# gmarcais/Jellyfish

Measured on AMD Instinct MI355X. Metric: k-mers/sec at k=21 canonical, 150 bp synthetic reads, bit-exact counts, higher is better.
Workload: dtype u64

## Files before the change

### jellyfish_amd/csrc/kernels.hip.hpp

```cpp
#pragma once
#include <hip/hip_runtime.h>
#include <stdint.h>
#include "kmer_core.hpp"

namespace jfgpu {

constexpr int kBlock = 256;
constexpr int kPerThread = kPerLane;
constexpr int kTilePos = kBlock * kPerThread;

enum Counter : int { CTR_FULL = 0, CTR_MERS = 1, CTR_OVF_FULL = 2, CTR_OVF_USED = 3, CTR_MISROUTED = 4, CTR_DIRECT = 5,
                     CTR_T_ITEMS = 6, CTR_T_QUEUED = 7 ,
                     CTR_PROF0 = 8 , CTR_COUNT = 12 };

#ifdef JFGPU_PHASE_PROF
__device__ unsigned long long g_phase_prof[24];
struct PhaseClk {
  long long acc[8] = {0, 0, 0, 0, 0, 0, 0, 0}; long long t;
  __device__ PhaseClk() { t = clock64(); }
  __device__ void mark(int i) { const long long n = clock64(); acc[i] += n - t; t = n; }
  __device__ void flush(int base) { if(threadIdx.x == 0) for(int i = 0; i < 8; ++i) if(acc[i]) atomicAdd(&g_phase_prof[base + i], (unsigned long long)acc[i]); }
};
#define JF_PHASE(pc, i) (pc).mark(i)
#define JF_PHASE_FLUSH(pc, base) (pc).flush(base)
// ... 4 lines not shown
#endif

struct DevBloom {
  uint32_t* data;
  uint64_t m;
  uint64_t recip;
  uint32_t nh;
  uint32_t nbytes;
  uint32_t kind;
  uint32_t pad_;
  const uint64_t* tbl1;
  const uint64_t* tbl2;
  uint64_t* cache;
  uint64_t cache_mask;
};

struct DevTable {
  TableGeom g;
  uint64_t* slots;
  const uint64_t* fwd_tbl;
  const uint64_t* inv_tbl;
  uint64_t* ovf_key;
  uint64_t* ovf_cnt;
  uint64_t ovf_mask;
  uint64_t* counters;
  uint32_t max_probe;
  DevBloom bloom;
  uint8_t* dirty;
};

#if defined(JFGPU_EMU)
__device__ __forceinline__ void lds_barrier() { __syncthreads(); }
#define JF_DYN_LDS(name) unsigned char* name = ::hip_emu::dyn_lds()
#else
__device__ __forceinline__ void lds_barrier() { asm volatile("s_waitcnt lgkmcnt(0)\n\ts_barrier" ::: "memory"); }
#define JF_DYN_LDS(name) extern __shared__ __align__(16) unsigned char name[]
#endif

__device__ inline bool bloom_admits(const DevBloom& B, uint64_t key);
__device__ inline uint32_t bloom_admit_mask(const DevBloom& B, const TableGeom& g, const LaneWords& L);

__device__ inline void ovf_add(const DevTable& T, uint64_t slot, uint64_t units) {
  const uint64_t want = slot + 1;
  uint64_t h = (slot * 0x9E3779B97F4A7C15ull) >> 20;
  for(uint64_t p = 0; p <= T.ovf_mask; ++p) {
    const uint64_t s = (h + p) & T.ovf_mask;
    unsigned long long old = atomicCAS((unsigned long long*)&T.ovf_key[s], 0ull, (unsigned long long)want);
    if(old == 0ull) atomicAdd((unsigned long long*)&T.counters[CTR_OVF_USED], 1ull);
    if(old == 0ull || old == want) {
      atomicAdd((unsigned long long*)&T.ovf_cnt[s], (unsigned long long)units);
      return;
    }
  }
  atomicAdd((unsigned long long*)&T.counters[CTR_OVF_FULL], 1ull);
}

__device__ inline uint64_t ovf_get(const DevTable& T, uint64_t slot) {
  const uint64_t want = slot + 1;
  uint64_t h = (slot * 0x9E3779B97F4A7C15ull) >> 20;
  for(uint64_t p = 0; p <= T.ovf_mask; ++p) {
    const uint64_t s = (h + p) & T.ovf_mask;
    const uint64_t k = T.ovf_key[s];
    if(k == 0) return 0;
    if(k == want) return T.ovf_cnt[s];
  }
  return 0;
}

__device__ inline uint64_t full_count(const DevTable& T, uint64_t word, uint64_t slot, bool have_ovf) {
// ... 892 lines not shown
```

### jellyfish_amd/csrc/kernels_bloom_part.hip.hpp

```cpp
#pragma once
#include "kernels_part.hip.hpp"
#include "kernels_p1ring.hip.hpp"
#include "kernels_bloom.hip.hpp"

namespace jfgpu {

constexpr uint32_t kBloomSegBits = 16;
constexpr uint32_t kBloomItemLow = kBloomSegBits + 3;
constexpr int kBloomPer = 10;
constexpr int kBloomChunk = kPBlock * kBloomPer;

struct BloomPart {
  uint32_t b1, b2;
  uint32_t n_seg;
  uint32_t pad_;
};

__device__ inline void bloom_item_direct(const DevBloom& B, const BloomPart& BP, uint32_t bucket, uint32_t item) {
  const uint64_t seg = ((uint64_t)bucket << BP.b2) | (item >> kBloomItemLow);
  const uint64_t byte = (seg << kBloomSegBits) | ((item >> 3) & 0xFFFFu);
  bloom_bump(B.data, byte, item & 7u);
}

struct BloomDirect {
// ... 132 lines not shown
                                                                   unsigned int* __restrict__ gcur, unsigned long long* __restrict__ tot,
                                                                   uint32_t* __restrict__ out, unsigned long long* __restrict__ mers) {
  p1_bloom_granule_body<NB, kBloomPer, false>(B, BP, g, base, lo, hi, cap, gcur, tot, out, mers);
}
template <int NB>
__global__ __launch_bounds__(kPBlock) __attribute__((amdgpu_waves_per_eu(8, 8)))
void p1_bloom_granule2_kernel(DevBloom B, BloomPart BP, TableGeom g, const uint8_t* __restrict__ base,
                              int64_t lo, int64_t hi, uint32_t cap,
                              unsigned int* __restrict__ gcur, unsigned long long* __restrict__ tot,
                              uint32_t* __restrict__ out, unsigned long long* __restrict__ mers) {
  p1_bloom_granule_body<NB, 5, true>(B, BP, g, base, lo, hi, cap, gcur, tot, out, mers);
}


constexpr uint32_t kBloomRingBytes = 256;
__device__ __attribute__((noinline)) void bloom_p1_item_direct_call(uint32_t* data, uint32_t b2, uint32_t bucket, uint32_t item) {
  const uint64_t seg = ((uint64_t)bucket << b2) | (item >> kBloomItemLow);
  const uint64_t byte = (seg << kBloomSegBits) | ((item >> 3) & 0xFFFFu);
  bloom_bump(data, byte, item & 7u);
}
struct BloomP1RingDirect {
  static constexpr bool kCountsDirect = false;
  uint32_t* data; uint32_t b2;
  __device__ void operator()(uint32_t bucket, uint64_t item, uint32_t cnt) const { for(uint32_t i = 0; i < cnt; ++i) bloom_p1_item_direct_call(data, b2, bucket, (uint32_t)item); }
};

template <int NB, int PER>
__global__ __launch_bounds__(kPBlock) void p1_bloom_ring_kernel(DevBloom B, BloomPart BP, TableGeom g, BloomP1RingDirect D, const uint8_t* __restrict__ base,
                                                                int64_t lo, int64_t hi, uint32_t cap,
                                                                unsigned int* __restrict__ gcur, unsigned long long* __restrict__ tot,
                                                                uint32_t* __restrict__ out, unsigned long long* __restrict__ mers,
                                                                uint64_t* __restrict__ strag, uint32_t* __restrict__ strag_n) {
  using R = Ring<uint32_t, kBloomRingBytes>;
  JF_DYN_LDS(s_dyn);
  const uint32_t nb = 1u << BP.b1;
  uint32_t* s_ring = reinterpret_cast<uint32_t*>(s_dyn);
  uint4* s_tn = reinterpret_cast<uint4*>(s_dyn + (size_t)nb * kBloomRingBytes + kBloomRingBytes);
  __shared__ uint32_t s_fill[kGranMaxB + 32];
  __shared__ uint32_t s_nstrag;
  __shared__ uint32_t s_codes[kPBlock + 2];
  __shared__ uint32_t s_inv[kPBlock + 2];
  const uint32_t t = threadIdx.x, lane = t & 63;
  const bool owner = t < nb;
  for(uint32_t i = t; i < B.nbytes * 32; i += blockDim.x) {
    const uint32_t j = i >> 4, v = i & 15u;
    const uint32_t at = (j >> 1) * 256 + ((j & 1) ? (v << 4) : v);
    const uint64_t a = B.tbl1[at], c = B.tbl2[at];
    s_tn[i] = make_uint4((uint32_t)a, (uint32_t)(a >> 32), (uint32_t)c, (uint32_t)(c >> 32));
  }
  ring_init<uint32_t, kBloomRingBytes>(s_ring, s_fill, nb, &s_nstrag);
  const uint32_t dump = nb * R::kSlots + (lane & (R::kSlots - 1));
  unsigned int* const gshort = gcur + nb;
  uint64_t* const my_strag = strag + (size_t)blockIdx.x * kStragPerBlock;
  const uint32_t k = g.k, rc_shift = 2 * (k - 1);
  const uint32_t sub_mask = (1u << BP.b2) - 1u;
  RingBooks Bk;
  if(owner) { Bk.nxt = atomicAdd(&gcur[t], kGran); Bk.nxt_asked = true; }
  uint32_t* const my_region = out + (uint64_t)t * cap;
  uint32_t my_mers = 0;
  auto straggler = [&](uint32_t b, uint32_t item, uint32_t cnt) {
    const uint32_t at = atomicAdd(&s_nstrag, 1u);
    if(at < kStragPerBlock) strag_store<uint32_t>(my_strag + at, b, item, cnt);
    else D(b, (uint64_t)item, cnt);
  };
  const int64_t n_tiles = (hi + kPTilePos - 1) / kPTilePos;
  TileRaw Rw = tile_fetch(base, (int64_t)blockIdx.x * kPTilePos, lo, hi);
  lds_barrier();
  for(int64_t tile = blockIdx.x; tile < n_tiles; tile += gridDim.x) {
    const LaneWords L = tile_stage(Rw, tile * kPTilePos, lo, hi, s_codes, s_inv);
    Rw = tile_fetch(base, (tile + gridDim.x) * kPTilePos, lo, hi);
    uint64_t fw = (((uint64_t)L.p2 << 32) | L.p1) & g.key_mask;
    uint64_t rc = revcomp64(fw, k);
    uint64_t smear = L.inv48;
    for(uint32_t s = 1; s < k; ) { const uint32_t step = s < k - s ? s : k - s; smear |= smear >> step; s += step; }
    const uint32_t vmask = ~(uint32_t)smear & 0xFFFFu;
    my_mers += (uint32_t)__popc(vmask);
#pragma unroll 1
    for(int j = 0; j < kPerLane; ++j) {
      const uint64_t c = (L.cur >> (2 * (15 - j))) & 3u;
      fw = ((fw << 2) | c) & g.key_mask;
      rc = (rc >> 2) | ((3ull - c) << rc_shift);
      const bool valid = (vmask >> (15 - j)) & 1u;
      const uint64_t key = (g.canonical && rc < fw) ? rc : fw;
      uint32_t a0 = 0, a1 = 0, c0 = 0, c1 = 0;
      constexpr int kNibs = NB ? 2 * NB : 16;
#pragma unroll
      for(int q = 0; q < kNibs; ++q)
        if(NB || (uint32_t)q < 2 * B.nbytes) { const uint4 e = s_tn[q * 16 + ((uint32_t)(key >> (4 * q)) & 15u)]; a0 ^= e.x; a1 ^= e.y; c0 ^= e.z; c1 ^= e.w; }
      uint64_t cell = bloom_mod(((uint64_t)a1 << 32) | a0, B.m, B.recip);
      const uint64_t inc = bloom_mod(((uint64_t)c1 << 32) | c0, B.m, B.recip);
      for(uint32_t h0 = 0; h0 < B.nh; h0 += PER) {
        uint32_t ea[PER], eo[PER], ei[PER];
#pragma unroll
        for(int e = 0; e < PER; ++e) {
          const bool on = valid && h0 + e < B.nh;
          uint64_t byte; uint32_t dig;
          divmod5(cell, byte, dig);
          const uint32_t seg = (uint32_t)(byte >> kBloomSegBits);
          const uint32_t b = seg >> BP.b2;
          ei[e] = ((seg & sub_mask) << kBloomItemLow) | ((uint32_t)(byte & 0xFFFFu) << 3) | dig;
          const uint32_t o = atomicAdd(&s_fill[on ? b : nb + (lane & 31u)], 1u);
          ea[e] = on ? b * R::kSlots : dump; eo[e] = on ? o : 0u;
          cell += inc; if(cell >= B.m) cell -= B.m;
        }
        uint32_t ghosts = 0;
#pragma unroll
        for(int e = 0; e < PER; ++e) {
          const uint32_t full = eo[e] & R::kFull;
          ghosts |= full;
          const uint32_t at = ea[e] + ((eo[e] + (eo[e] >> 16)) & (R::kSlots - 1));
          s_ring[full ? dump : at] = ei[e];
        }
        if(ghosts) {
#pragma unroll 1
          for(int e = 0; e < PER; ++e) if(eo[e] & R::kFull) straggler(ea[e] / R::kSlots, ei[e], 1u);
        }
        lds_barrier();
        wave_prio<3>();
        if(owner) ring_flush<uint32_t, false, kBloomRingBytes>(s_ring, s_fill, t, false, Bk, my_region, cap, gcur, gshort, straggler);
        wave_prio<0>();
#ifdef JFGPU_BLOOM_P1_BAR2
        lds_barrier();
#endif
      }
    }
  }
  lds_barrier();
  if(owner) { ring_flush<uint32_t, false, kBloomRingBytes>(s_ring, s_fill, t, true, Bk, my_region, cap, gcur, gshort, straggler); ring_finish<uint32_t>(Bk, t, my_region, cap, gshort, tot); }
  lds_barrier();
  if(t == 0) strag_n[blockIdx.x] = s_nstrag < kStragPerBlock ? s_nstrag : kStragPerBlock;
  uint64_t w = my_mers;
  for(int o = 32; o > 0; o >>= 1) w += __shfl_down(w, o, 64);
  if((threadIdx.x & 63) == 0 && w) atomicAdd(mers, (unsigned long long)w);
}

__device__ inline void bloom_lds_bump(uint32_t* s_seg, uint32_t item) {
  const uint32_t off = (item >> 3) & 0xFFFFu, dig = item & 7u;
  uint32_t* w = s_seg + (off >> 2);
  const uint32_t sh = 8 * (off & 3);
  const uint32_t add = bloom_pow3(dig) << sh;
  uint32_t old = *w;
  while(true) {
    if(bloom_digit((old >> sh) & 0xFFu, dig) >= 2) return;
    const uint32_t seen = atomicCAS(w, old, old + add);
    if(seen == old) return;
    old = seen;
  }
}
// ... 53 lines not shown
```

### jellyfish_amd/csrc/kernels_p1ring.hip.hpp

```cpp
#pragma once
#include <type_traits>
#include "kernels_part.hip.hpp"

namespace jfgpu {

template <int P> __device__ __forceinline__ void wave_prio() {
#if defined(__HIP_DEVICE_COMPILE__)
  __builtin_amdgcn_s_setprio(P);
#endif
}

__device__ __forceinline__ uint32_t adm_to_vmask(uint32_t adm) {
  uint32_t r = 0;
#pragma unroll
  for(int j = 0; j < 16; ++j) r |= ((adm >> j) & 1u) << (15 - j);
  return r;
}


constexpr uint32_t kStragPerBlock = 16384;

template <typename ITEM, uint32_t RB = 128> struct Ring {
  static constexpr uint32_t kSlots = RB / sizeof(ITEM);
  static constexpr uint32_t kUnit = 64 / sizeof(ITEM);
  static constexpr uint32_t kChunk = 16 / sizeof(ITEM);
  static constexpr uint32_t kFull = 0xFFFFu & ~(kSlots - 1);
  static constexpr uint32_t kWords = sizeof(ITEM) <= 4 ? 1 : 1 + sizeof(ITEM) / 8;
  __device__ static uint32_t first_fill(uint32_t b) { return ((kChunk * b) & (kSlots - 1)) << 16; }
};

template <typename ITEM> __device__ __forceinline__ uint32_t chunk_hole_key(const uint4& v) {
  if constexpr(sizeof(ITEM) == 4) { const uint32_t a = v.x > v.y ? v.x : v.y, c = v.z > v.w ? v.z : v.w; return a > c ? a : c; }
  else if constexpr(sizeof(ITEM) == 8) { const uint32_t a = v.x & v.y, c = v.z & v.w; return a > c ? a : c; }
  else return v.x & v.y & v.z & v.w;
}
template <typename ITEM, typename F> __device__ __forceinline__ void chunk_items(const uint4& v, F&& f) {
  if constexpr(sizeof(ITEM) == 4) { f((ITEM)v.x); f((ITEM)v.y); f((ITEM)v.z); f((ITEM)v.w); }
  else if constexpr(sizeof(ITEM) == 8) { f((ITEM)(((uint64_t)v.y << 32) | v.x)); f((ITEM)(((uint64_t)v.w << 32) | v.z)); }
  else f((ITEM)(((unsigned __int128)(((uint64_t)v.w << 32) | v.z) << 64) | (((uint64_t)v.y << 32) | v.x)));
}

template <typename ITEM> __device__ __forceinline__ void strag_store(uint64_t* rec, uint32_t b, ITEM item, uint32_t cnt) {
  const uint64_t meta = ((uint64_t)(cnt < 255u ? cnt : 255u) << 56) | ((uint64_t)(b & 0xFFFFFFu) << 32);
  if constexpr(sizeof(ITEM) == 4) rec[0] = meta | (uint32_t)item;
  else if constexpr(sizeof(ITEM) == 8) { rec[0] = meta; rec[1] = (uint64_t)item; }
  else { rec[0] = meta; rec[1] = (uint64_t)item; rec[2] = (uint64_t)(item >> 64); }
}
template <typename ITEM> __device__ __forceinline__ void strag_load(const uint64_t* rec, uint32_t& b, ITEM& item, uint32_t& cnt) {
  const uint64_t meta = rec[0];
  b = (uint32_t)(meta >> 32) & 0xFFFFFFu; cnt = (uint32_t)(meta >> 56);
  if constexpr(sizeof(ITEM) == 4) item = (ITEM)(uint32_t)meta;
  else if constexpr(sizeof(ITEM) == 8) item = (ITEM)rec[1];
  else item = (ITEM)(((unsigned __int128)rec[2] << 64) | rec[1]);
}

struct RingBooks { uint32_t gpos = 0, room = 0, nxt = 0, stored = 0; bool nxt_asked = false, exhausted = false; };

template <typename ITEM, bool OWNED = false, uint32_t RB = 128, typename STRAG>
__device__ __forceinline__ void ring_flush(ITEM* s_ring, uint32_t* s_fill, uint32_t t, bool all, RingBooks& B, ITEM* my_region, uint32_t cap,
                                           unsigned int* gcur, unsigned int* gshort, STRAG&& straggler) {
  using R = Ring<ITEM, RB>;
  const ITEM hole = (ITEM)~(ITEM)0;
  const uint32_t w = s_fill[t];
  uint32_t cnt = w & 0xFFFFu; if(cnt > R::kSlots) cnt = R::kSlots;
  const uint32_t rb = (w >> 16) & (R::kSlots - 1);
  uint32_t units = cnt / R::kUnit; if(all && (cnt % R::kUnit)) ++units;
  uint32_t nout = 0;
  for(uint32_t s = 0; s < units; ++s) {
    uint4 v[4];
    const uint32_t s0 = (rb + s * R::kUnit) & (R::kSlots - 1);
#pragma unroll
    for(int q = 0; q < 4; ++q) v[q] = *reinterpret_cast<const uint4*>(s_ring + t * R::kSlots + ((s0 + R::kChunk * q) & (R::kSlots - 1)));
    if(!all) {
      uint32_t mx = 0;
#pragma unroll
      for(int q = 0; q < 4; ++q) { const uint32_t a = chunk_hole_key<ITEM>(v[q]); mx = mx > a ? mx : a; }
      if(mx == 0xFFFFFFFFu) break;
    }
    if constexpr(!OWNED) {
    if(B.room == 0 && B.nxt_asked) {
      if((uint64_t)B.nxt + kGran <= cap) { B.gpos = B.nxt; B.room = kGran; }
      else { B.exhausted = true; if(B.nxt < cap) atomicMax(&gshort[t], cap - B.nxt); }
      B.nxt_asked = false;
    }
    if(B.room == 0 && !B.exhausted) {
      const uint32_t r0 = atomicAdd(&gcur[t], kGran);
      if((uint64_t)r0 + kGran <= cap) { B.gpos = r0; B.room = kGran; }
      else { B.exhausted = true; if(r0 < cap) atomicMax(&gshort[t], cap - r0); }
    }
    }
    if(B.room) {
      uint4* dst = reinterpret_cast<uint4*>(my_region + B.gpos);
#pragma unroll
      for(int q = 0; q < 4; ++q) dst[q] = v[q];
      const uint32_t real = cnt - s * R::kUnit < R::kUnit ? cnt - s * R::kUnit : R::kUnit;
      B.gpos += OWNED ? real : R::kUnit; B.room -= R::kUnit; B.stored += real;
    } else {
#pragma unroll
      for(int q = 0; q < 4; ++q) chunk_items<ITEM>(v[q], [&](ITEM x) { if(x != hole) straggler(t, x, 1u); });
    }
#pragma unroll
    for(int q = 0; q < 4; ++q)
      *reinterpret_cast<uint4*>(s_ring + t * R::kSlots + ((s0 + R::kChunk * q) & (R::kSlots - 1))) = make_uint4(0xFFFFFFFFu, 0xFFFFFFFFu, 0xFFFFFFFFu, 0xFFFFFFFFu);
    ++nout;
  }
  if constexpr(!OWNED) { if(!all && !B.nxt_asked && !B.exhausted && B.room < R::kSlots) { B.nxt = atomicAdd(&gcur[t], kGran); B.nxt_asked = true; } }
  uint32_t expect = w;
  while(nout || (expect & 0xFFFFu) > R::kSlots) {
    uint32_t c = expect & 0xFFFFu; if(c > R::kSlots) c = R::kSlots;
    const uint32_t taken = nout * R::kUnit < c ? nout * R::kUnit : c;
    const uint32_t neww = ((((expect >> 16) + nout * R::kUnit) & 0xFFFFu) << 16) | (c - taken);
    const uint32_t old = atomicCAS(&s_fill[t], expect, neww);
    if(old == expect) break;
    expect = old;
  }
}

template <typename ITEM, uint32_t RB = 128>
__device__ __forceinline__ void ring_init(ITEM* s_ring, uint32_t* s_fill, uint32_t nb, uint32_t* s_nstrag) {
  using R = Ring<ITEM, RB>;
  for(uint32_t j = threadIdx.x; j < nb; j += blockDim.x) s_fill[j] = R::first_fill(j);
  uint4* r4 = reinterpret_cast<uint4*>(s_ring);
  for(uint32_t j = threadIdx.x; j < nb * (RB / 16) + RB / 16; j += blockDim.x) r4[j] = make_uint4(0xFFFFFFFFu, 0xFFFFFFFFu, 0xFFFFFFFFu, 0xFFFFFFFFu);
  if(threadIdx.x == 0) *s_nstrag = 0;
}

template <typename ITEM>
__device__ __forceinline__ void ring_finish(const RingBooks& B, uint32_t t, ITEM* my_region, uint32_t cap, unsigned int* gshort, unsigned long long* tot) {
  const ITEM hole = (ITEM)~(ITEM)0;
  for(uint32_t r = 0; r < B.room; ++r) my_region[B.gpos + r] = hole;
  if(B.nxt_asked) {
    if((uint64_t)B.nxt + kGran <= cap) { for(uint32_t r = 0; r < kGran; ++r) my_region[B.nxt + r] = hole; }
    else if(B.nxt < cap) atomicMax(&gshort[t], cap - B.nxt);
  }
  if(tot && B.stored) atomicAdd(&tot[t], (unsigned long long)B.stored);
}

struct OneWordDirect {
  static constexpr bool kCountsDirect = true;
  const DevTable* Tm; uint32_t b2; int returning;
  __device__ void operator()(uint32_t b, uint64_t item, uint32_t cnt) const { item_direct_call(Tm, b2, b, item, cnt, returning); }
};
struct RouteListDirect {
  static constexpr bool kCountsDirect = false;
  StragList SL;
  __device__ void operator()(uint32_t b, uint64_t item, uint32_t cnt) const {
    for(uint32_t i = 0; i < cnt; ++i) { const unsigned long long at = atomicAdd(SL.n, 1ull); if(at < SL.cap) SL.rec[at] = ((uint64_t)b << 32) | (uint32_t)item; }
  }
};

template <typename ITEM, bool BLOOM, int NB, int CANON, typename DIRECT = OneWordDirect>
__global__ __launch_bounds__(kPBlock) void p1_ring_kernel(DevTable T, DIRECT D, PartGeom P, const uint8_t* __restrict__ base,
                                                          int64_t lo, int64_t hi, uint32_t cap,
                                                          unsigned int* __restrict__ gcur,
                                                          unsigned long long* __restrict__ tot,
                                                          ITEM* __restrict__ out,
                                                          uint64_t* __restrict__ strag, uint32_t* __restrict__ strag_n) {
  using R = Ring<ITEM>;
  constexpr int RP = sizeof(ITEM) == 4 ? 8 : 4;
  JF_DYN_LDS(s_dyn);
  ITEM* s_ring = reinterpret_cast<ITEM*>(s_dyn);
  __shared__ uint64_t s_fwd[NB < 0 ? 1 : 8 * 256];
  __shared__ uint32_t s_fill[kGranMaxB + 32];
  __shared__ uint32_t s_nstrag;
  __shared__ uint32_t s_codes[kPBlock + 2];
  __shared__ uint32_t s_inv[kPBlock + 2];
  const TableGeom& g = T.g;
  const uint32_t nb = 1u << P.b1;
  const uint32_t t = threadIdx.x, lane = t & 63;
  const bool owner = t < nb;
  const ITEM hole = (ITEM)~(ITEM)0;
  if constexpr(NB >= 0) load_tables_lds(s_fwd, T.fwd_tbl, g.nbytes);
  ring_init<ITEM>(s_ring, s_fill, nb, &s_nstrag);
  const uint32_t dump = nb * R::kSlots + (lane & (R::kSlots - 1));
  [[maybe_unused]] const uint32_t xs_hi_mask = g.lsize_g > 32 ? (g.lsize_g >= 64 ? 0xFFFFFFFFu : ((1u << (g.lsize_g - 32)) - 1u)) : 0u;
  unsigned int* const gshort = gcur + nb;
  uint64_t* const my_strag = strag + (size_t)blockIdx.x * kStragPerBlock * R::kWords;
  const uint32_t k = g.k, bshift = g.lsize_l - P.b1;
  const uint32_t rc_shift = 2 * (k - 1);
  const uint32_t rest_mask = P.rest_shift >= 32 ? 0xFFFFFFFFu : ((1u << P.rest_shift) - 1u);
  RingBooks B;
  if(owner) { B.nxt = atomicAdd(&gcur[t], kGran); B.nxt_asked = true; }
  ITEM* const my_region = out + (uint64_t)t * cap;
  uint32_t my_mers = 0, my_direct = 0;

  auto straggler = [&](uint32_t b, ITEM item, uint32_t cnt) {
    const uint32_t at = atomicAdd(&s_nstrag, 1u);
    if(at < kStragPerBlock) strag_store<ITEM>(my_strag + (size_t)at * R::kWords, b, item, cnt);
    else { D(b, (uint64_t)item, cnt); ++my_direct; }
  };

  const int64_t n_tiles = (hi + kPTilePos - 1) / kPTilePos;
  TileRaw Rw = tile_fetch(base, (int64_t)blockIdx.x * kPTilePos, lo, hi);
  lds_barrier();
  [[maybe_unused]] PhaseClk pc;
  for(int64_t tile = blockIdx.x; tile < n_tiles; tile += gridDim.x) {
    const LaneWords L = tile_stage(Rw, tile * kPTilePos, lo, hi, s_codes, s_inv);
    Rw = tile_fetch(base, (tile + gridDim.x) * kPTilePos, lo, hi);
    JF_PHASE(pc, 0);
    const uint32_t adm = BLOOM ? bloom_admit_mask(T.bloom, g, L) : 0xFFFFu;
    uint64_t fw = (((uint64_t)L.p2 << 32) | L.p1) & g.key_mask;
    uint64_t rc = revcomp64(fw, k);
    uint64_t smear = L.inv48;
    for(uint32_t s = 1; s < k; ) { const uint32_t step = s < k - s ? s : k - s; smear |= smear >> step; s += step; }
    const uint32_t rawmask = ~(uint32_t)smear & 0xFFFFu;
    const uint32_t vmask = BLOOM ? (rawmask & adm_to_vmask(adm)) : rawmask;
    my_mers += (uint32_t)__popc(rawmask);
    auto rounds = [&](auto runs_tag) {
    constexpr bool RUNS = decltype(runs_tag)::value;
    uint64_t pk = 0; uint32_t pv = 0, run = 0;
#pragma unroll 1
    for(int j0 = 0; j0 < kPerLane; j0 += RP) {
      constexpr int NE = RUNS ? RP + 1 : RP;
      uint32_t ea[NE], eo[NE]; ITEM ei[NE];
      [[maybe_unused]] uint32_t spm = 0;
#pragma unroll
      for(int e = 0; e < NE; ++e) { ea[e] = dump; ei[e] = 0; eo[e] = 0; }
      auto emit = [&](int e, uint64_t key, uint32_t cnt, bool on) {
        uint32_t b; ITEM item;
        if constexpr(NB == kHashXS && sizeof(ITEM) == 4) {
          uint32_t ylo, yhi;
          xs_hash_halves<false>((uint32_t)key, (uint32_t)(key >> 32), xs_hi_mask, ylo, yhi);
          b = funnel_r(yhi, ylo, bshift) & (nb - 1);
          item = ((ylo & rest_mask) << g.rem_bits) | ((uint32_t)(key >> 32) >> (g.lsize_g - 32));
        } else {
          const uint64_t pos = NB < 0 ? xs_hash(key, g.lsize_g, g.key_bits) : hash_tables_t<(NB < 0 ? 0 : NB)>(s_fwd, key, g.nbytes);
          b = (uint32_t)(pos >> bshift) & (nb - 1);
          if constexpr(sizeof(ITEM) == 4) item = (((uint32_t)pos & rest_mask) << g.rem_bits) | (uint32_t)(key >> g.lsize_g);
          else item = make_item<ITEM>(g, P, key, pos & g.local_mask);
        }
        const bool special = on && (item == hole || cnt > 1);
        const bool normal = on && !special;
#ifndef JFGPU_P1_LATE_SPECIAL
        if(special) straggler(b, item, cnt);
        const uint32_t o = atomicAdd(&s_fill[normal ? b : nb + (lane & 31u)], 1u);
        ea[e] = normal ? b * R::kSlots : dump; ei[e] = item; eo[e] = normal ? o : 0u;
#else
        const uint32_t o = atomicAdd(&s_fill[normal ? b : nb + (lane & 31u)], 1u);
        spm |= special ? 1u << e : 0u;
        ea[e] = on ? b * R::kSlots : dump; ei[e] = item; eo[e] = normal ? o : special ? (R::kFull | ((cnt < 0xFFFFu ? cnt : 0xFFFFu) << 16)) : 0u;
#endif
      };
#ifndef JFGPU_P1_OLD_EXTRACT
      const uint32_t cur_r = L.cur << (2 * j0), ncur_r = ~cur_r, vm_r = vmask << j0;
#endif
#pragma unroll
      for(int e = 0; e < RP; ++e) {
#ifndef JFGPU_P1_OLD_EXTRACT
        const uint32_t c = (cur_r >> (2 * (15 - e))) & 3u, nc = (ncur_r >> (2 * (15 - e))) & 3u;
        const uint32_t v = vm_r & (1u << (15 - e));
#else
        const int j = j0 + e;
        const uint32_t c = (L.cur >> (2 * (15 - j))) & 3u, nc = 3u - c;
        const uint32_t v = vmask & (1u << (15 - j));
#endif
        if constexpr(NB >= 5 || NB == kHashXS) {
          const uint32_t flo = (uint32_t)fw, fhi = (uint32_t)(fw >> 32), rlo = (uint32_t)rc, rhi = (uint32_t)(rc >> 32);
          fw = ((uint64_t)(funnel_r(fhi, flo, 30) & (uint32_t)(g.key_mask >> 32)) << 32) | ((flo << 2) | c);
          rc = ((uint64_t)((rhi >> 2) | (nc << (rc_shift - 32))) << 32) | funnel_r(rhi, rlo, 2);
        } else {
          fw = ((fw << 2) | c) & g.key_mask;
          rc = (rc >> 2) | ((uint64_t)nc << rc_shift);
        }
        const uint64_t key = ((CANON == 1 || (CANON == 2 && g.canonical)) && rc < fw) ? rc : fw;
        if constexpr(RUNS) {
#ifdef JFGPU_P1_NO_RUNS
          const bool same = false;
#else
          const bool same = v && pv && key == pk;
#endif
          emit(e, pk, run, pv && !same);
          run = same ? run + 1 : 1;
          pk = key; pv = v;
        } else emit(e, key, 1u, v != 0);
      }
      if constexpr(RUNS) { if(j0 + RP >= kPerLane) { emit(NE - 1, pk, run, pv != 0); pv = 0; } }
      uint32_t ghosts = 0;
#pragma unroll
      for(int e = 0; e < NE; ++e) {
        const uint32_t full = eo[e] & R::kFull;
        ghosts |= full;
        const uint32_t at = ea[e] + ((eo[e] + (eo[e] >> 16)) & (R::kSlots - 1));
        s_ring[full ? dump : at] = ei[e];
      }
      if(ghosts) {
#pragma unroll 1
#ifndef JFGPU_P1_LATE_SPECIAL
        for(int e = 0; e < NE; ++e) {
          uint32_t a = 0, o = 0; ITEM it = 0;
#pragma unroll
          for(int q = 0; q < NE; ++q) if(q == e) { a = ea[q]; o = eo[q]; it = ei[q]; }
          if(o & R::kFull) straggler(a / R::kSlots, it, 1u);
        }
#else
        for(int e = 0; e < NE; ++e) if(eo[e] & R::kFull) straggler(ea[e] / R::kSlots, ei[e], ((spm >> e) & 1u) ? eo[e] >> 16 : 1u);
#endif
      }
      JF_PHASE(pc, 1);
      lds_barrier();
      JF_PHASE(pc, 2);
#ifndef JFGPU_P1_NO_FLUSH_PRIO
      wave_prio<3>();
#endif
      if(owner) ring_flush<ITEM>(s_ring, s_fill, t, false, B, my_region, cap, gcur, gshort, straggler);
#ifndef JFGPU_P1_NO_FLUSH_PRIO
      wave_prio<0>();
#endif
      JF_PHASE(pc, 3);
    }
    };
    bool may_run = k < 14;
    {
      const uint32_t hc = L.cur ^ (L.cur >> 2), hp = L.p1 ^ (L.p1 >> 2);
      may_run = may_run || (hc & 0x3FFFu) == 0 || ((hc >> 16) & 0x3FFFu) == 0 || (hp & 0x3FFFu) == 0;
    }
#ifdef JFGPU_P1_ALWAYS_RUNS
    may_run = true;
#endif
    if(__ballot(may_run) != 0ull) rounds(std::true_type{}); else rounds(std::false_type{});
  }
  lds_barrier();
  if(owner) { ring_flush<ITEM>(s_ring, s_fill, t, true, B, my_region, cap, gcur, gshort, straggler); ring_finish<ITEM>(B, t, my_region, cap, gshort, tot); }
  lds_barrier();
  if(t == 0) strag_n[blockIdx.x] = s_nstrag < kStragPerBlock ? s_nstrag : kStragPerBlock;
  JF_PHASE(pc, 4);
  JF_PHASE_FLUSH(pc, 0);
  if(DIRECT::kCountsDirect && my_direct) atomicAdd((unsigned long long*)&T.counters[CTR_DIRECT], (unsigned long long)my_direct);
  uint64_t w = my_mers;
  for(int o = 32; o > 0; o >>= 1) w += __shfl_down(w, o, 64);
// ... 9 lines not shown
  uint32_t my_direct = 0;
  for(uint32_t l = blockIdx.x; l < n_lists; l += gridDim.x) {
    const uint32_t n = strag_n[l];
    const uint64_t* rec = strag + (size_t)l * list_cap * R::kWords;
    for(uint32_t i = threadIdx.x; i < n; i += blockDim.x) {
      uint32_t b, cnt; ITEM item;
      strag_load<ITEM>(rec + (size_t)i * R::kWords, b, item, cnt);
      if(cnt == 1 && item != (ITEM)~(ITEM)0) {
        const uint32_t at = atomicAdd(&gcur[b], 1u);
        if(at < cap) { out[(uint64_t)b * cap + at] = item; if(tot) atomicAdd(&tot[b], 1ull); continue; }
        atomicMin(&gcur[b], cap);
      }
      D(b, item, cnt);
      ++my_direct;
    }
  }
  if(ctr_direct && my_direct) atomicAdd(ctr_direct, (unsigned long long)my_direct);
}

constexpr uint32_t kP2StragPerBlock = 2048;

struct P2RingDirect {
  const DevTable* Tm; uint32_t b2; uint32_t dest_shift; int returning;
  __device__ void operator()(uint32_t dest, uint64_t item, uint32_t cnt) const { item_direct_call(Tm, b2, dest >> dest_shift, item, cnt, returning); }
};

template <typename DIRECT>
__global__ __launch_bounds__(kPBlock) void p2_ring_kernel(DIRECT D, uint32_t b2e, uint32_t tag_bits, SegList S, uint32_t cap,
                                                          unsigned int* __restrict__ gcur, unsigned int* __restrict__ gshort,
                                                          uint32_t* __restrict__ out, uint32_t bucket0, unsigned long long* __restrict__ tot,
                                                          uint64_t* __restrict__ strag, uint32_t* __restrict__ strag_n, unsigned long long* __restrict__ ctr_direct) {
  using R = Ring<uint32_t>;
  constexpr int RP = 8;
  JF_DYN_LDS(s_dyn);
  uint32_t* s_ring = reinterpret_cast<uint32_t*>(s_dyn);
  __shared__ uint32_t s_fill[kGranMaxB];
  __shared__ uint32_t s_nstrag;
  const uint32_t nb = 1u << b2e;
  const uint32_t bucket = bucket0 + blockIdx.y;
  const uint32_t dest0 = bucket * nb;
  const uint32_t t = threadIdx.x, lane = t & 63;
  const bool owner = t < nb;
  const uint32_t hole = 0xFFFFFFFFu;
  ring_init<uint32_t>(s_ring, s_fill, nb, &s_nstrag);
  const uint32_t dump = nb * R::kSlots + (lane & (R::kSlots - 1));
  unsigned int* const gc = gcur + dest0;
  unsigned int* const gs = gshort + dest0;
  const uint32_t list = blockIdx.y * gridDim.x + blockIdx.x;
  uint64_t* const my_strag = strag + (size_t)list * kP2StragPerBlock;
  RingBooks B;
  if(owner) { B.nxt = atomicAdd(&gc[t], kGran); B.nxt_asked = true; }
  uint32_t* const my_region = out + ((uint64_t)dest0 + t) * cap;
  uint32_t my_direct = 0;
  auto straggler = [&](uint32_t d, uint32_t item, uint32_t cnt) {
    const uint32_t at = atomicAdd(&s_nstrag, 1u);
    if(at < kP2StragPerBlock) strag_store<uint32_t>(my_strag + at, dest0 + d, item, cnt);
    else { D(dest0 + d, (uint64_t)item, cnt); ++my_direct; }
  };
  auto flush = [&](bool all) { if(owner) ring_flush<uint32_t>(s_ring, s_fill, t, all, B, my_region, cap, gc, gs, straggler); };
  lds_barrier();
  uint32_t seg = 0; uint64_t my_a = 0, my_b = 0;
  const uint32_t* src = nullptr;
  auto next_seg = [&]() -> bool {
    for(; seg < S.n; ++seg) {
      const uint64_t a0 = seg_lo(S, seg, bucket), b0 = seg_hi(S, seg, bucket);
      const uint64_t len4 = (b0 - a0 + 3) / 4;
      const uint64_t per4 = (len4 + gridDim.x - 1) / gridDim.x;
      const uint64_t q0 = (uint64_t)blockIdx.x * per4, q1 = q0 + per4;
      const uint64_t e1 = a0 + 4 * (q1 < len4 ? q1 : len4);
      my_a = a0 + 4 * (q0 < len4 ? q0 : len4); my_b = e1 < b0 ? e1 : b0;
      src = reinterpret_cast<const uint32_t*>(S.items[seg]);
      if(my_a < my_b) return true;
    }
    return false;
  };
  constexpr uint64_t RS = (uint64_t)kPBlock * RP;
  auto load_full = [&](uint64_t r0, uint32_t (&it)[RP]) {
#pragma unroll
    for(int h = 0; h < RP / 4; ++h) {
      const uint4 v = *reinterpret_cast<const uint4*>(src + r0 + (uint64_t)h * kPBlock * 4 + 4 * (uint64_t)t);
      it[4 * h] = v.x; it[4 * h + 1] = v.y; it[4 * h + 2] = v.z; it[4 * h + 3] = v.w;
    }
  };
  auto load_partial = [&](uint64_t r0, uint32_t (&it)[RP]) {
#pragma unroll
    for(int h = 0; h < RP / 4; ++h) {
      const uint64_t i = r0 + (uint64_t)h * kPBlock * 4 + 4 * (uint64_t)t;
      uint4 v = make_uint4(hole, hole, hole, hole);
      if(i + 4 <= my_b) v = *reinterpret_cast<const uint4*>(src + i);
      else if(i < my_b) { v.x = src[i]; if(i + 1 < my_b) v.y = src[i + 1]; if(i + 2 < my_b) v.z = src[i + 2]; }
      it[4 * h] = v.x; it[4 * h + 1] = v.y; it[4 * h + 2] = v.z; it[4 * h + 3] = v.w;
    }
  };
  auto process = [&](const uint32_t (&it)[RP]) {
    uint32_t ea[RP], eo[RP];
#pragma unroll
    for(int e = 0; e < RP; ++e) {
      ea[e] = dump; eo[e] = 0;
      if(it[e] != hole) { const uint32_t d = (it[e] >> tag_bits) & (nb - 1); ea[e] = d * R::kSlots; eo[e] = atomicAdd(&s_fill[d], 1u); }
    }
    uint32_t ghosts = 0;
#pragma unroll
    for(int e = 0; e < RP; ++e) {
      const uint32_t full = eo[e] & R::kFull;
      ghosts |= full;
      const uint32_t at = ea[e] + ((eo[e] + (eo[e] >> 16)) & (R::kSlots - 1));
      s_ring[full ? dump : at] = it[e];
    }
    if(ghosts) {
#pragma unroll 1
      for(int e = 0; e < RP; ++e) if(eo[e] & R::kFull) straggler(ea[e] / R::kSlots, it[e], 1u);
    }
    lds_barrier();
    flush(false);
    lds_barrier();
  };
  for(bool have = next_seg(); have; ++seg, have = next_seg()) {
    uint64_t r0 = my_a;
    const uint64_t n_full = (my_b - my_a) / RS;
    if(n_full) {
      uint32_t nx[RP];
      load_full(r0, nx);
#pragma unroll 1
      for(uint64_t k = 0; k < n_full; ++k) {
        uint32_t it[RP];
#pragma unroll
        for(int e = 0; e < RP; ++e) it[e] = nx[e];
        r0 += RS;
        load_full(k + 1 < n_full ? r0 : my_a, nx);
        process(it);
      }
    }
    if(r0 < my_b) { uint32_t it[RP]; load_partial(r0, it); process(it); }
  }
  lds_barrier();
  flush(true);
  if(owner) ring_finish<uint32_t>(B, t, my_region, cap, gs, tot ? tot + dest0 : nullptr);
  lds_barrier();
  if(t == 0) strag_n[list] = s_nstrag < kP2StragPerBlock ? s_nstrag : kP2StragPerBlock;
  if(my_direct) atomicAdd(ctr_direct, (unsigned long long)my_direct);
}

template <typename ITEM, int NV, typename DIRECT, int PD = 1>
__global__ __launch_bounds__(kPBlock) void p2_ring_roles_kernel(DIRECT D, uint32_t b2e, uint32_t tag_bits, SegList S, uint32_t cap,
                                                                unsigned int* __restrict__ gcur, ITEM* __restrict__ out, uint32_t bucket0,
                                                                uint64_t* __restrict__ strag, uint32_t* __restrict__ strag_n, unsigned long long* __restrict__ ctr_direct) {
  using R = Ring<ITEM>;
  constexpr int VPI = (int)R::kChunk;
  constexpr int RP = NV * VPI;
  constexpr uint32_t kHalf = kPBlock / 2;
  constexpr uint64_t RS = (uint64_t)kHalf * RP;
  JF_DYN_LDS(s_dyn);
  ITEM* s_ring = reinterpret_cast<ITEM*>(s_dyn);
  __shared__ uint32_t s_fill[kGranMaxB];
  __shared__ uint32_t s_nstrag;
  const uint32_t nb = 1u << b2e;
  const uint32_t bucket = bucket0 + blockIdx.x;
  const uint32_t dest0 = bucket * nb;
  const uint32_t t = threadIdx.x, lane = t & 63;
  const bool storer = t < kHalf;
  const ITEM hole = (ITEM)~(ITEM)0;
  ring_init<ITEM>(s_ring, s_fill, nb, &s_nstrag);
  const uint32_t dump = nb * R::kSlots + (lane & (R::kSlots - 1));
  uint64_t* const my_strag = strag + (size_t)blockIdx.x * kP2StragPerBlock * R::kWords;
  uint32_t my_direct = 0;
  auto straggler = [&](uint32_t d, ITEM item, uint32_t cnt) {
    const uint32_t at = atomicAdd(&s_nstrag, 1u);
    if(at < kP2StragPerBlock) strag_store<ITEM>(my_strag + (size_t)at * R::kWords, dest0 + d, item, cnt);
    else { D(dest0 + d, item, cnt); ++my_direct; }
  };
  lds_barrier();
  auto seg_bounds = [&](uint32_t seg, uint64_t& a, uint64_t& b) { a = seg_lo(S, seg, bucket); b = seg_hi(S, seg, bucket); };
  if(storer) {
    const uint32_t d0 = t, d1 = t + kHalf;
    const bool has0 = d0 < nb, has1 = d1 < nb;
    RingBooks B0, B1;
    B0.room = B1.room = cap & ~(R::kUnit - 1);
    ITEM* const r0p = out + ((uint64_t)dest0 + d0) * cap;
    ITEM* const r1p = out + ((uint64_t)dest0 + d1) * cap;
    auto flush = [&](bool all) {
      if(has0) ring_flush<ITEM, true>(s_ring, s_fill, d0, all, B0, r0p, cap, gcur, gcur, straggler);
      if(has1) ring_flush<ITEM, true>(s_ring, s_fill, d1, all, B1, r1p, cap, gcur, gcur, straggler);
    };
    for(uint32_t seg = 0; seg < S.n; ++seg) {
      uint64_t a, b; seg_bounds(seg, a, b);
      const uint64_t rounds = (b - a + RS - 1) / RS;
#pragma unroll 1
      for(uint64_t r = 0; r < rounds; ++r) { lds_barrier(); flush(false); }
    }
    lds_barrier();
    flush(true);
    if(has0) gcur[dest0 + d0] = B0.gpos;
    if(has1) gcur[dest0 + d1] = B1.gpos;
  } else {
    const uint32_t l = t - kHalf;
    for(uint32_t seg = 0; seg < S.n; ++seg) {
// ... 1 lines not shown
      const ITEM* src = reinterpret_cast<const ITEM*>(S.items[seg]);
      auto load_full = [&](uint64_t r0, ITEM (&it)[RP]) {
#pragma unroll
        for(int h = 0; h < NV; ++h) {
          const uint4 v = *reinterpret_cast<const uint4*>(src + r0 + (uint64_t)h * kHalf * VPI + (uint64_t)VPI * l);
          int q = 0;
          chunk_items<ITEM>(v, [&](ITEM x) { it[VPI * h + q] = x; ++q; });
        }
      };
      auto load_partial = [&](uint64_t r0, ITEM (&it)[RP]) {
#pragma unroll
        for(int h = 0; h < NV; ++h) {
          const uint64_t i = r0 + (uint64_t)h * kHalf * VPI + (uint64_t)VPI * l;
#pragma unroll
          for(int q = 0; q < VPI; ++q) it[VPI * h + q] = i + q < b ? src[i + q] : hole;
        }
      };
      auto load_exact = [&](uint64_t r0, ITEM (&it)[RP]) {
#pragma unroll 1
        for(int h = 0; h < NV; ++h) {
          const uint64_t i = r0 + (uint64_t)h * kHalf * VPI + (uint64_t)VPI * l;
#pragma unroll
          for(int q = 0; q < VPI; ++q) {
            ITEM x = hole;
            if(i + q < b) { x = src[i + q]; if(x == hole) straggler((uint32_t)(x >> tag_bits) & (nb - 1), x, 1u); }
            it[VPI * h + q] = x;
          }
        }
      };
      auto append = [&](const ITEM (&it)[RP]) {
        uint32_t ea[RP], eo[RP];
#pragma unroll
        for(int e = 0; e < RP; ++e) {
          ea[e] = dump; eo[e] = 0;
          if(it[e] != hole) { const uint32_t d = (uint32_t)(it[e] >> tag_bits) & (nb - 1); ea[e] = d * R::kSlots; eo[e] = atomicAdd(&s_fill[d], 1u); }
        }
        uint32_t ghosts = 0;
#pragma unroll
        for(int e = 0; e < RP; ++e) {
          const uint32_t full = eo[e] & R::kFull;
          ghosts |= full;
          const uint32_t at = ea[e] + ((eo[e] + (eo[e] >> 16)) & (R::kSlots - 1));
          s_ring[full ? dump : at] = it[e];
        }
        if(ghosts) {
#pragma unroll 1
          for(int e = 0; e < RP; ++e) if(eo[e] & R::kFull) straggler(ea[e] / R::kSlots, it[e], 1u);
        }
        lds_barrier();
      };
      uint64_t r0 = a;
      if(S.sh[seg] == 0) {
#pragma unroll 1
        for(; r0 < b; r0 += RS) { ITEM it[RP]; load_exact(r0, it); append(it); }
        continue;
      }
      const uint64_t n_full = (b - a) / RS;
      if(n_full) {
        ITEM nx[PD][RP];
#pragma unroll
        for(int d = 0; d < PD; ++d) load_full((uint64_t)d < n_full ? a + (uint64_t)d * RS : a, nx[d]);
        uint64_t k = 0;
#pragma unroll 1
        for(; k + PD <= n_full; k += PD) {
#pragma unroll
          for(int d = 0; d < PD; ++d) {
            ITEM it[RP];
#pragma unroll
            for(int e = 0; e < RP; ++e) it[e] = nx[d][e];
            const uint64_t nxt = k + d + PD;
            load_full(nxt < n_full ? a + nxt * RS : a, nx[d]);
            append(it);
          }
        }
#pragma unroll
        for(int d = 0; d < PD - 1; ++d)
          if(k + d < n_full) append(nx[d]);
        r0 = a + n_full * RS;
      }
      if(r0 < b) { ITEM it[RP]; load_partial(r0, it); append(it); }
// ... 10 lines not shown
```

Baseline: 15.83 billion.

## Re-encode ring fill words as byte offsets with outstanding-count carry field

After: 15.59 billion. 0.984x the previous value.

```diff
diff --git a/jellyfish_amd/csrc/kernels.hip.hpp b/jellyfish_amd/csrc/kernels.hip.hpp
--- a/jellyfish_amd/csrc/kernels.hip.hpp
+++ b/jellyfish_amd/csrc/kernels.hip.hpp
@@ -60,9 +60,11 @@
 #if defined(JFGPU_EMU)
 __device__ __forceinline__ void lds_barrier() { __syncthreads(); }
 #define JF_DYN_LDS(name) unsigned char* name = ::hip_emu::dyn_lds()
+#define JF_DYN_LDS_RINGS(name) JF_DYN_LDS(name)
 #else
 __device__ __forceinline__ void lds_barrier() { asm volatile("s_waitcnt lgkmcnt(0)\n\ts_barrier" ::: "memory"); }
 #define JF_DYN_LDS(name) extern __shared__ __align__(16) unsigned char name[]
+#define JF_DYN_LDS_RINGS(name) extern __shared__ __align__(256) unsigned char name[]
 #endif
 
 __device__ inline bool bloom_admits(const DevBloom& B, uint64_t key);
diff --git a/jellyfish_amd/csrc/kernels_bloom_part.hip.hpp b/jellyfish_amd/csrc/kernels_bloom_part.hip.hpp
--- a/jellyfish_amd/csrc/kernels_bloom_part.hip.hpp
+++ b/jellyfish_amd/csrc/kernels_bloom_part.hip.hpp
@@ -188,7 +188,7 @@
                                                                 uint32_t* __restrict__ out, unsigned long long* __restrict__ mers,
                                                                 uint64_t* __restrict__ strag, uint32_t* __restrict__ strag_n) {
   using R = Ring<uint32_t, kBloomRingBytes>;
-  JF_DYN_LDS(s_dyn);
+  JF_DYN_LDS_RINGS(s_dyn);
   const uint32_t nb = 1u << BP.b1;
   uint32_t* s_ring = reinterpret_cast<uint32_t*>(s_dyn);
   uint4* s_tn = reinterpret_cast<uint4*>(s_dyn + (size_t)nb * kBloomRingBytes + kBloomRingBytes);
@@ -205,7 +205,8 @@
     s_tn[i] = make_uint4((uint32_t)a, (uint32_t)(a >> 32), (uint32_t)c, (uint32_t)(c >> 32));
   }
   ring_init<uint32_t, kBloomRingBytes>(s_ring, s_fill, nb, &s_nstrag);
-  const uint32_t dump = nb * R::kSlots + (lane & (R::kSlots - 1));
+  ring_spare_reset(s_fill, nb);
+  const uint32_t ring0 = R::origin(s_ring), dump0 = ring0 + nb * kBloomRingBytes, dump = dump0 + (lane & (R::kSlots - 1)) * R::kStep;
   unsigned int* const gshort = gcur + nb;
   uint64_t* const my_strag = strag + (size_t)blockIdx.x * kStragPerBlock;
   const uint32_t k = g.k, rc_shift = 2 * (k - 1);
@@ -225,6 +226,7 @@
   for(int64_t tile = blockIdx.x; tile < n_tiles; tile += gridDim.x) {
     const LaneWords L = tile_stage(Rw, tile * kPTilePos, lo, hi, s_codes, s_inv);
     Rw = tile_fetch(base, (tile + gridDim.x) * kPTilePos, lo, hi);
+    ring_spare_reset(s_fill, nb);
     uint64_t fw = (((uint64_t)L.p2 << 32) | L.p1) & g.key_mask;
     uint64_t rc = revcomp64(fw, k);
     uint64_t smear = L.inv48;
@@ -255,21 +257,16 @@
           const uint32_t seg = (uint32_t)(byte >> kBloomSegBits);
           const uint32_t b = seg >> BP.b2;
           ei[e] = ((seg & sub_mask) << kBloomItemLow) | ((uint32_t)(byte & 0xFFFFu) << 3) | dig;
-          const uint32_t o = atomicAdd(&s_fill[on ? b : nb + (lane & 31u)], 1u);
-          ea[e] = on ? b * R::kSlots : dump; eo[e] = on ? o : 0u;
+          eo[e] = atomicAdd(&s_fill[on ? b : nb + (lane & 31u)], on ? R::kAppend : R::kStep);
+          ea[e] = ring0 + (on ? b : nb) * kBloomRingBytes;
           cell += inc; if(cell >= B.m) cell -= B.m;
         }
-        uint32_t ghosts = 0;
-#pragma unroll
-        for(int e = 0; e < PER; ++e) {
-          const uint32_t full = eo[e] & R::kFull;
-          ghosts |= full;
-          const uint32_t at = ea[e] + ((eo[e] + (eo[e] >> 16)) & (R::kSlots - 1));
-          s_ring[full ? dump : at] = ei[e];
-        }
+        bool ghosts = false;
+#pragma unroll
+        for(int e = 0; e < PER; ++e) ghosts |= R::put(s_ring, ea[e], eo[e], dump, ei[e]);
         if(ghosts) {
 #pragma unroll 1
-          for(int e = 0; e < PER; ++e) if(eo[e] & R::kFull) straggler(ea[e] / R::kSlots, ei[e], 1u);
+          for(int e = 0; e < PER; ++e) if(eo[e] >= R::kFullWord && ea[e] != dump0) straggler((ea[e] - ring0) / kBloomRingBytes, ei[e], 1u);
         }
         lds_barrier();
         wave_prio<3>();
diff --git a/jellyfish_amd/csrc/kernels_p1ring.hip.hpp b/jellyfish_amd/csrc/kernels_p1ring.hip.hpp
--- a/jellyfish_amd/csrc/kernels_p1ring.hip.hpp
+++ b/jellyfish_amd/csrc/kernels_p1ring.hip.hpp
@@ -24,9 +24,29 @@
   static constexpr uint32_t kSlots = RB / sizeof(ITEM);
   static constexpr uint32_t kUnit = 64 / sizeof(ITEM);
   static constexpr uint32_t kChunk = 16 / sizeof(ITEM);
-  static constexpr uint32_t kFull = 0xFFFFu & ~(kSlots - 1);
   static constexpr uint32_t kWords = sizeof(ITEM) <= 4 ? 1 : 1 + sizeof(ITEM) / 8;
-  __device__ static uint32_t first_fill(uint32_t b) { return ((kChunk * b) & (kSlots - 1)) << 16; }
+  static_assert(sizeof(ITEM) <= 8, "a round of 16-byte items appends more than 2^17 bytes to one ring: widen the carry field first");
+  static constexpr uint32_t kStep = (uint32_t)sizeof(ITEM);
+  static constexpr uint32_t kMask = RB - kStep;
+  static constexpr uint32_t kOutShift = 17;
+  static constexpr uint32_t kAppend = (1u << kOutShift) | kStep;
+  static constexpr uint32_t kFullWord = kSlots << kOutShift;
+  __device__ static uint32_t first_fill(uint32_t b) { return (16u * b) & (RB - 1); }
+  __device__ static uint32_t outstanding(uint32_t w) { return w >> kOutShift; }
+  __device__ static ITEM* at(ITEM* s_ring, uint32_t byte) { return reinterpret_cast<ITEM*>(reinterpret_cast<unsigned char*>(s_ring) + byte); }
+#if defined(__HIP_DEVICE_COMPILE__) && !defined(JFGPU_EMU)
+  typedef __attribute__((address_space(3))) ITEM LdsItem;
+  __device__ static __forceinline__ uint32_t origin(ITEM* s_ring) { return (uint32_t)(uintptr_t)(LdsItem*)s_ring; }
+  __device__ static __forceinline__ void store(ITEM*, uint32_t addr, ITEM x) { *(LdsItem*)(uintptr_t)addr = x; }
+#else
+  __device__ static uint32_t origin(ITEM*) { return 0; }
+  __device__ static void store(ITEM* s_ring, uint32_t addr, ITEM x) { *at(s_ring, addr) = x; }
+#endif
+  __device__ static __forceinline__ bool put(ITEM* s_ring, uint32_t ring, uint32_t o, uint32_t dump, ITEM x) {
+    const bool full = o >= kFullWord;
+    store(s_ring, full ? dump : (ring | (o & kMask)), x);
+    return full;
+  }
 };
 
 template <typename ITEM> __device__ __forceinline__ uint32_t chunk_hole_key(const uint4& v) {
@@ -62,15 +82,15 @@
   using R = Ring<ITEM, RB>;
   const ITEM hole = (ITEM)~(ITEM)0;
   const uint32_t w = s_fill[t];
-  uint32_t cnt = w & 0xFFFFu; if(cnt > R::kSlots) cnt = R::kSlots;
-  const uint32_t rb = (w >> 16) & (R::kSlots - 1);
+  uint32_t cnt = R::outstanding(w); if(cnt > R::kSlots) cnt = R::kSlots;
+  const uint32_t tail = (w - R::outstanding(w) * R::kStep) & (RB - 1);
   uint32_t units = cnt / R::kUnit; if(all && (cnt % R::kUnit)) ++units;
   uint32_t nout = 0;
   for(uint32_t s = 0; s < units; ++s) {
     uint4 v[4];
-    const uint32_t s0 = (rb + s * R::kUnit) & (R::kSlots - 1);
-#pragma unroll
-    for(int q = 0; q < 4; ++q) v[q] = *reinterpret_cast<const uint4*>(s_ring + t * R::kSlots + ((s0 + R::kChunk * q) & (R::kSlots - 1)));
+    const uint32_t s0 = tail + s * 64u;
+#pragma unroll
+    for(int q = 0; q < 4; ++q) v[q] = *reinterpret_cast<const uint4*>(R::at(s_ring, t * RB + ((s0 + 16u * q) & (RB - 1))));
     if(!all) {
       uint32_t mx = 0;
 #pragma unroll
@@ -101,15 +121,17 @@
     }
 #pragma unroll
     for(int q = 0; q < 4; ++q)
-      *reinterpret_cast<uint4*>(s_ring + t * R::kSlots + ((s0 + R::kChunk * q) & (R::kSlots - 1))) = make_uint4(0xFFFFFFFFu, 0xFFFFFFFFu, 0xFFFFFFFFu, 0xFFFFFFFFu);
+      *reinterpret_cast<uint4*>(R::at(s_ring, t * RB + ((s0 + 16u * q) & (RB - 1)))) = make_uint4(0xFFFFFFFFu, 0xFFFFFFFFu, 0xFFFFFFFFu, 0xFFFFFFFFu);
     ++nout;
   }
   if constexpr(!OWNED) { if(!all && !B.nxt_asked && !B.exhausted && B.room < R::kSlots) { B.nxt = atomicAdd(&gcur[t], kGran); B.nxt_asked = true; } }
   uint32_t expect = w;
-  while(nout || (expect & 0xFFFFu) > R::kSlots) {
-    uint32_t c = expect & 0xFFFFu; if(c > R::kSlots) c = R::kSlots;
+  while(nout || R::outstanding(expect) > R::kSlots) {
+    const uint32_t eo = R::outstanding(expect);
+    const uint32_t c = eo > R::kSlots ? R::kSlots : eo;
     const uint32_t taken = nout * R::kUnit < c ? nout * R::kUnit : c;
-    const uint32_t neww = ((((expect >> 16) + nout * R::kUnit) & 0xFFFFu) << 16) | (c - taken);
+    const uint32_t p = eo > R::kSlots ? tail : expect;
+    const uint32_t neww = ((c - taken) << R::kOutShift) | (p & (RB - 1));
     const uint32_t old = atomicCAS(&s_fill[t], expect, neww);
     if(old == expect) break;
     expect = old;
@@ -124,6 +146,7 @@
   for(uint32_t j = threadIdx.x; j < nb * (RB / 16) + RB / 16; j += blockDim.x) r4[j] = make_uint4(0xFFFFFFFFu, 0xFFFFFFFFu, 0xFFFFFFFFu, 0xFFFFFFFFu);
   if(threadIdx.x == 0) *s_nstrag = 0;
 }
+__device__ __forceinline__ void ring_spare_reset(uint32_t* s_fill, uint32_t nb) { if(threadIdx.x < 32) s_fill[nb + threadIdx.x] = 0; }
 
 template <typename ITEM>
 __device__ __forceinline__ void ring_finish(const RingBooks& B, uint32_t t, ITEM* my_region, uint32_t cap, unsigned int* gshort, unsigned long long* tot) {
@@ -158,7 +181,7 @@
                                                           uint64_t* __restrict__ strag, uint32_t* __restrict__ strag_n) {
   using R = Ring<ITEM>;
   constexpr int RP = sizeof(ITEM) == 4 ? 8 : 4;
-  JF_DYN_LDS(s_dyn);
+  JF_DYN_LDS_RINGS(s_dyn);
   ITEM* s_ring = reinterpret_cast<ITEM*>(s_dyn);
   __shared__ uint64_t s_fwd[NB < 0 ? 1 : 8 * 256];
   __shared__ uint32_t s_fill[kGranMaxB + 32];
@@ -172,7 +195,11 @@
   const ITEM hole = (ITEM)~(ITEM)0;
   if constexpr(NB >= 0) load_tables_lds(s_fwd, T.fwd_tbl, g.nbytes);
   ring_init<ITEM>(s_ring, s_fill, nb, &s_nstrag);
-  const uint32_t dump = nb * R::kSlots + (lane & (R::kSlots - 1));
+  ring_spare_reset(s_fill, nb);
+  const uint32_t ring0 = R::origin(s_ring);
+  const uint32_t dump0 = ring0 + nb * R::kSlots * R::kStep;
+  const uint32_t dump_off = (lane & (R::kSlots - 1)) * R::kStep;
+  const uint32_t dump = dump0 + dump_off;
   [[maybe_unused]] const uint32_t xs_hi_mask = g.lsize_g > 32 ? (g.lsize_g >= 64 ? 0xFFFFFFFFu : ((1u << (g.lsize_g - 32)) - 1u)) : 0u;
   unsigned int* const gshort = gcur + nb;
   uint64_t* const my_strag = strag + (size_t)blockIdx.x * kStragPerBlock * R::kWords;
@@ -197,6 +224,7 @@
   for(int64_t tile = blockIdx.x; tile < n_tiles; tile += gridDim.x) {
     const LaneWords L = tile_stage(Rw, tile * kPTilePos, lo, hi, s_codes, s_inv);
     Rw = tile_fetch(base, (tile + gridDim.x) * kPTilePos, lo, hi);
+    ring_spare_reset(s_fill, nb);
     JF_PHASE(pc, 0);
     const uint32_t adm = BLOOM ? bloom_admit_mask(T.bloom, g, L) : 0xFFFFu;
     uint64_t fw = (((uint64_t)L.p2 << 32) | L.p1) & g.key_mask;
@@ -213,9 +241,8 @@
     for(int j0 = 0; j0 < kPerLane; j0 += RP) {
       constexpr int NE = RUNS ? RP + 1 : RP;
       uint32_t ea[NE], eo[NE]; ITEM ei[NE];
-      [[maybe_unused]] uint32_t spm = 0;
-#pragma unroll
-      for(int e = 0; e < NE; ++e) { ea[e] = dump; ei[e] = 0; eo[e] = 0; }
+#pragma unroll
+      for(int e = 0; e < NE; ++e) { ea[e] = dump0; ei[e] = 0; eo[e] = dump_off; }
       auto emit = [&](int e, uint64_t key, uint32_t cnt, bool on) {
         uint32_t b; ITEM item;
         if constexpr(NB == kHashXS && sizeof(ITEM) == 4) {
@@ -231,15 +258,9 @@
         }
         const bool special = on && (item == hole || cnt > 1);
         const bool normal = on && !special;
-#ifndef JFGPU_P1_LATE_SPECIAL
         if(special) straggler(b, item, cnt);
-        const uint32_t o = atomicAdd(&s_fill[normal ? b : nb + (lane & 31u)], 1u);
-        ea[e] = normal ? b * R::kSlots : dump; ei[e] = item; eo[e] = normal ? o : 0u;
-#else
-        const uint32_t o = atomicAdd(&s_fill[normal ? b : nb + (lane & 31u)], 1u);
-        spm |= special ? 1u << e : 0u;
-        ea[e] = on ? b * R::kSlots : dump; ei[e] = item; eo[e] = normal ? o : special ? (R::kFull | ((cnt < 0xFFFFu ? cnt : 0xFFFFu) << 16)) : 0u;
-#endif
+        const uint32_t o = atomicAdd(&s_fill[normal ? b : nb + (lane & 31u)], normal ? R::kAppend : R::kStep);
+        ea[e] = ring0 + (normal ? b : nb) * (R::kSlots * R::kStep); ei[e] = item; eo[e] = o;
       };
 #ifndef JFGPU_P1_OLD_EXTRACT
       const uint32_t cur_r = L.cur << (2 * j0), ncur_r = ~cur_r, vm_r = vmask << j0;
@@ -275,26 +296,17 @@
         } else emit(e, key, 1u, v != 0);
       }
       if constexpr(RUNS) { if(j0 + RP >= kPerLane) { emit(NE - 1, pk, run, pv != 0); pv = 0; } }
-      uint32_t ghosts = 0;
-#pragma unroll
-      for(int e = 0; e < NE; ++e) {
-        const uint32_t full = eo[e] & R::kFull;
-        ghosts |= full;
-        const uint32_t at = ea[e] + ((eo[e] + (eo[e] >> 16)) & (R::kSlots - 1));
-        s_ring[full ? dump : at] = ei[e];
-      }
+      bool ghosts = false;
+#pragma unroll
+      for(int e = 0; e < NE; ++e) ghosts |= R::put(s_ring, ea[e], eo[e], dump, ei[e]);
       if(ghosts) {
 #pragma unroll 1
-#ifndef JFGPU_P1_LATE_SPECIAL
         for(int e = 0; e < NE; ++e) {
           uint32_t a = 0, o = 0; ITEM it = 0;
 #pragma unroll
           for(int q = 0; q < NE; ++q) if(q == e) { a = ea[q]; o = eo[q]; it = ei[q]; }
-          if(o & R::kFull) straggler(a / R::kSlots, it, 1u);
-        }
-#else
-        for(int e = 0; e < NE; ++e) if(eo[e] & R::kFull) straggler(ea[e] / R::kSlots, ei[e], ((spm >> e) & 1u) ? eo[e] >> 16 : 1u);
-#endif
+          if(o >= R::kFullWord && a != dump0) straggler((a - ring0) / (R::kSlots * R::kStep), it, 1u);
+        }
       }
       JF_PHASE(pc, 1);
       lds_barrier();
@@ -370,7 +382,7 @@
                                                           uint64_t* __restrict__ strag, uint32_t* __restrict__ strag_n, unsigned long long* __restrict__ ctr_direct) {
   using R = Ring<uint32_t>;
   constexpr int RP = 8;
-  JF_DYN_LDS(s_dyn);
+  JF_DYN_LDS_RINGS(s_dyn);
   uint32_t* s_ring = reinterpret_cast<uint32_t*>(s_dyn);
   __shared__ uint32_t s_fill[kGranMaxB];
   __shared__ uint32_t s_nstrag;
@@ -381,7 +393,7 @@
   const bool owner = t < nb;
   const uint32_t hole = 0xFFFFFFFFu;
   ring_init<uint32_t>(s_ring, s_fill, nb, &s_nstrag);
-  const uint32_t dump = nb * R::kSlots + (lane & (R::kSlots - 1));
+  const uint32_t ring0 = R::origin(s_ring), dump0 = ring0 + nb * R::kSlots * R::kStep, dump_off = (lane & (R::kSlots - 1)) * R::kStep, dump = dump0 + dump_off;
   unsigned int* const gc = gcur + dest0;
   unsigned int* const gs = gshort + dest0;
   const uint32_t list = blockIdx.y * gridDim.x + blockIdx.x;
@@ -434,20 +446,15 @@
     uint32_t ea[RP], eo[RP];
 #pragma unroll
     for(int e = 0; e < RP; ++e) {
-      ea[e] = dump; eo[e] = 0;
-      if(it[e] != hole) { const uint32_t d = (it[e] >> tag_bits) & (nb - 1); ea[e] = d * R::kSlots; eo[e] = atomicAdd(&s_fill[d], 1u); }
-    }
-    uint32_t ghosts = 0;
-#pragma unroll
-    for(int e = 0; e < RP; ++e) {
-      const uint32_t full = eo[e] & R::kFull;
-      ghosts |= full;
-      const uint32_t at = ea[e] + ((eo[e] + (eo[e] >> 16)) & (R::kSlots - 1));
-      s_ring[full ? dump : at] = it[e];
-    }
+      ea[e] = dump0; eo[e] = dump_off;
+      if(it[e] != hole) { const uint32_t d = (it[e] >> tag_bits) & (nb - 1); ea[e] = ring0 + d * (R::kSlots * R::kStep); eo[e] = atomicAdd(&s_fill[d], R::kAppend); }
+    }
+    bool ghosts = false;
+#pragma unroll
+    for(int e = 0; e < RP; ++e) ghosts |= R::put(s_ring, ea[e], eo[e], dump, it[e]);
     if(ghosts) {
 #pragma unroll 1
-      for(int e = 0; e < RP; ++e) if(eo[e] & R::kFull) straggler(ea[e] / R::kSlots, it[e], 1u);
+      for(int e = 0; e < RP; ++e) if(eo[e] >= R::kFullWord) straggler((ea[e] - ring0) / (R::kSlots * R::kStep), it[e], 1u);
     }
     lds_barrier();
     flush(false);
@@ -488,7 +495,7 @@
   constexpr int RP = NV * VPI;
   constexpr uint32_t kHalf = kPBlock / 2;
   constexpr uint64_t RS = (uint64_t)kHalf * RP;
-  JF_DYN_LDS(s_dyn);
+  JF_DYN_LDS_RINGS(s_dyn);
   ITEM* s_ring = reinterpret_cast<ITEM*>(s_dyn);
   __shared__ uint32_t s_fill[kGranMaxB];
   __shared__ uint32_t s_nstrag;
@@ -499,7 +506,7 @@
   const bool storer = t < kHalf;
   const ITEM hole = (ITEM)~(ITEM)0;
   ring_init<ITEM>(s_ring, s_fill, nb, &s_nstrag);
-  const uint32_t dump = nb * R::kSlots + (lane & (R::kSlots - 1));
+  const uint32_t ring0 = R::origin(s_ring), dump0 = ring0 + nb * R::kSlots * R::kStep, dump_off = (lane & (R::kSlots - 1)) * R::kStep, dump = dump0 + dump_off;
   uint64_t* const my_strag = strag + (size_t)blockIdx.x * kP2StragPerBlock * R::kWords;
   uint32_t my_direct = 0;
   auto straggler = [&](uint32_t d, ITEM item, uint32_t cnt) {
@@ -567,20 +574,15 @@
         uint32_t ea[RP], eo[RP];
 #pragma unroll
         for(int e = 0; e < RP; ++e) {
-          ea[e] = dump; eo[e] = 0;
-          if(it[e] != hole) { const uint32_t d = (uint32_t)(it[e] >> tag_bits) & (nb - 1); ea[e] = d * R::kSlots; eo[e] = atomicAdd(&s_fill[d], 1u); }
-        }
-        uint32_t ghosts = 0;
-#pragma unroll
-        for(int e = 0; e < RP; ++e) {
-          const uint32_t full = eo[e] & R::kFull;
-          ghosts |= full;
-          const uint32_t at = ea[e] + ((eo[e] + (eo[e] >> 16)) & (R::kSlots - 1));
-          s_ring[full ? dump : at] = it[e];
-        }
+          ea[e] = dump0; eo[e] = dump_off;
+          if(it[e] != hole) { const uint32_t d = (uint32_t)(it[e] >> tag_bits) & (nb - 1); ea[e] = ring0 + d * (R::kSlots * R::kStep); eo[e] = atomicAdd(&s_fill[d], R::kAppend); }
+        }
+        bool ghosts = false;
+#pragma unroll
+        for(int e = 0; e < RP; ++e) ghosts |= R::put(s_ring, ea[e], eo[e], dump, it[e]);
         if(ghosts) {
 #pragma unroll 1
-          for(int e = 0; e < RP; ++e) if(eo[e] & R::kFull) straggler(ea[e] / R::kSlots, it[e], 1u);
+          for(int e = 0; e < RP; ++e) if(eo[e] >= R::kFullWord) straggler((ea[e] - ring0) / (R::kSlots * R::kStep), it[e], 1u);
         }
         lds_barrier();
       };
```
